# keyber/Single-Image-Super-Resolution

Measured on AMD Instinct MI355X. Metric: HR patches/sec (x2 generator fwd+bwd, LR 96x96 -> SR 192x192), higher is better.
Workload: dtype f32; 1 GPU; SRGAN x2 generator (16 blocks, 64 features, spectral norm) fwd+bwd+Adam with bicubic LR degradation and pixel-MSE x10, per-GPU batch 16 HR 192x192 patches (LR 96x96 -> SR 192x192): the north star's headline. BASELINE.json's metric string "96^2 crops, x4" is configs.cfg3 of this line. Single build: fp32.; per_gpu_batch=16, hr=192, lr=96, parallelism=dp1, hip_graph=True

## Files before the change

### single-image-super-resolution_amd/csrc/conv_trunk_f32.hip

```cpp
#include "sisr_dev.h"
#include "sisr_bf16_stage.h"
#include "sisr_instr.h"

typedef unsigned cf_u32x4 __attribute__((ext_vector_type(4)));

#include <type_traits>

#define CF_TH 8
#define CF_TW 16
#define CF_IH (CF_TH + 2)
#define CF_IW (CF_TW + 2)
#define CF_NPIX (CF_IH * CF_IW)
#define CF_PSF 36
#define CF_HALO_BYTES (CF_NPIX * CF_PSF * 4)
#define CF_WROW 36
#define CF_WCHUNK_BYTES (9 * 32 * CF_WROW * 4)
#define CF_ITEMS ((CF_NPIX * 8 + 255) / 256)
#define CF_THREADS 512
#define CF_KROWP 100
#define CF_PS 33

SISR_TRACE_BUFFER(sisr_cftrace, 512, 128)
#define CFT(k) SISR_TRACE_STAMP(sisr_cftrace, threadIdx.x == 0, blockIdx.x, k, 64, wall_clock64())
#define CFTP(k) SISR_TRACE_STAMP(sisr_cftrace, threadIdx.x == 256, blockIdx.x, 64 + (k), 128, wall_clock64())
SISR_TRACE_BUFFER(sisr_cfclk, 512, 2)
#define CFTC(k) SISR_TRACE_STAMP(sisr_cfclk, threadIdx.x == 0, blockIdx.x, (k) - 60, 2, clock64())

struct CTrunkF32Args {
    const float *x1, *x2;
    float* x_out;
    BnFinArgs fin;
    const float *pa, *pb, *pd, *ps, *pt;
    const float* slope_p; float slope;
    const float* wpk;
    const void* wimg;
    const float* bias;
    const float* res;
    float* y;
    float *stat_part, *cnt_part;
    const float *bnb_x, *bnb_scale, *bnb_shift, *bnb_mean, *bnb_invstd, *bnb_slope_p;
    float bnb_slope; int bnb_act;
    float* bnb_part;
    int N, H, W;
    int tiles_x, per_img, total, streams;
    uint32_t m_tiles_x, m_per_img;
    int glog, cout_pad, shuffle;
    int xsc, xph;
};

__device__ __forceinline__ __amdgpu_buffer_rsrc_t cf_rsrc(const void* p, unsigned bytes) {
    return __builtin_amdgcn_make_buffer_rsrc(const_cast<void*>(p), 0, (int)bytes, 0x00020000);
}

__device__ __forceinline__ void cf_split2(float v0, float v1, unsigned& hw, unsigned& lw) {
    const f32x2 v = {v0, v1};
    hw = __builtin_bit_cast(unsigned, __builtin_convertvector(v, bf16x2));
    const f32x2 r = {v0 - __uint_as_float(hw << 16), v1 - __uint_as_float(hw & 0xFFFF0000u)};
    lw = __builtin_bit_cast(unsigned, __builtin_convertvector(r, bf16x2));
}

template <int PRO, bool SPLIT>
__global__ void __launch_bounds__(CF_THREADS, 2) conv_trunk_f32_kernel(const CTrunkF32Args a) {
    extern __shared__ __attribute__((aligned(16))) unsigned char lds[];
    unsigned char* halo0 = lds + 2 * CF_WCHUNK_BYTES;
    float* red = reinterpret_cast<float*>(halo0 + 2 * CF_HALO_BYTES);

    const int tid = threadIdx.x, lane = tid & 63;
    const int wave = __builtin_amdgcn_readfirstlane(tid >> 6);
    const bool consumer = wave < 4;
    const int l31 = lane & 31, kk = lane >> 5;
    const bool xcd = (a.streams & 7) == 0;
    const int hc = xcd ? (blockIdx.x >> 3) & ((1 << a.glog) - 1) : blockIdx.x & ((1 << a.glog) - 1);
    const int stream = xcd ? (blockIdx.x & 7) | ((blockIdx.x >> (3 + a.glog)) << 3) : blockIdx.x >> a.glog;
    const unsigned tbytes = (unsigned)a.N * (unsigned)a.H * (unsigned)a.W * 256u;
    constexpr bool TWO = PRO == SISR_PRO_BNBWD || PRO == SISR_PRO_BNACT_BWD || PRO == SISR_PRO_RES_AFFINE || PRO == SISR_PRO_ACT_BWD;
    constexpr bool SUM = PRO == SISR_PRO_RES_AFFINE;
    auto tile_coords = [&](int T, int& n, int& ty, int& tx) {
        n = fdiv(T, a.m_per_img);
        const int rem = T - n * a.per_img;
        ty = fdiv(rem, a.m_tiles_x);
        tx = rem - ty * a.tiles_x;
    };

    CFT(0);
    CFTC(60);
    float* kfin = red + 4 * 32 * 3;
    const bool fin = (PRO == SISR_PRO_AFFINE_ACT || PRO == SISR_PRO_RES_AFFINE) && a.fin.stat != nullptr;
    if (fin) bn_finalize_in_kernel(a.fin, reinterpret_cast<double*>(lds), kfin, blockIdx.x == 0);
    auto fill_weights = [&]() {
        float* wl = reinterpret_cast<float*>(lds);
        if (a.wimg != nullptr) {
            constexpr int UNITS = 2 * 9 * 32 * CF_WROW / 4;
            constexpr int W_IT16 = (UNITS + CF_THREADS - 1) / CF_THREADS;
            const cf_u32x4* src = reinterpret_cast<const cf_u32x4*>(a.wimg) + hc * UNITS;
            cf_u32x4 wv16[W_IT16];
#pragma unroll
            for (int it = 0; it < W_IT16; ++it) {
                const int u = tid + it * CF_THREADS;
                wv16[it] = u < UNITS ? src[u] : cf_u32x4{0u, 0u, 0u, 0u};
            }
#pragma unroll
            for (int it = 0; it < W_IT16; ++it) {
                const int u = tid + it * CF_THREADS;
                if (u < UNITS) reinterpret_cast<cf_u32x4*>(wl)[u] = wv16[it];
            }
            return;
        }
        constexpr int W_IT = 2 * 9 * 32 * 32 / CF_THREADS;
        float wv[W_IT];
#pragma unroll
        for (int it = 0; it < W_IT; ++it) {
            const int e = tid + it * CF_THREADS;
            const int ci = e & 31, s = (e >> 5) % 3, t2 = (e >> 5) / 3;
            const int co = t2 & 31, qr = t2 >> 5;
            wv[it] = a.wpk[((int64_t)qr * a.cout_pad + 32 * hc + co) * CF_KROWP + s * CF_PS + ci];
        }
#pragma unroll
        for (int it = 0; it < W_IT; ++it) {
            const int e = tid + it * CF_THREADS;
            const int ci = e & 31, s = (e >> 5) % 3, t2 = (e >> 5) / 3;
            const int co = t2 & 31, qr = t2 >> 5;
            const int q = qr / 3, r = qr - 3 * q;
            if constexpr (SPLIT) {
                const float vo = __shfl_xor(wv[it], 1);
                const bool odd = ci & 1;
                unsigned hw, lw;
                cf_split2(odd ? vo : wv[it], odd ? wv[it] : vo, hw, lw);
                reinterpret_cast<unsigned*>(wl)[((q * 9 + r * 3 + s) * 32 + co) * CF_WROW + (odd ? 16 : 0) + (ci >> 1)] = odd ? lw : hw;
            } else {
                wl[((q * 9 + r * 3 + s) * 32 + co) * CF_WROW + ci] = wv[it];
            }
        }
    };

    const int n_mine = stream < a.total ? (a.total - stream + a.streams - 1) / a.streams : 0;
    const int n_stages = 2 * n_mine;

    if (!consumer) {
        const int pt = tid & 255, quad = tid & 7, m0 = pt >> 3;
        const int tiles_y = a.per_img / a.tiles_x;
        const float slope = PRO != SISR_PRO_NONE ? (a.slope_p ? a.slope_p[0] : a.slope) : 1.f;
        f32x4 ka[2], kb[2], kd[2], ks[2], kt[2];
        int rel[CF_ITEMS];
        unsigned flags = 0;
#pragma unroll
        for (int k = 0; k < CF_ITEMS; ++k) {
            const int px = m0 + 32 * k;
            const int py = px / CF_IW, pxx = px - py * CF_IW;
            rel[k] = ((py - 1) * a.xsc * a.xsc * a.W + (pxx - 1) * a.xsc) * 256 + quad * 16;
            const unsigned f = (py == 0 ? 1u : 0u) | (py == CF_IH - 1 ? 2u : 0u) | (pxx == 0 ? 4u : 0u) | (pxx == CF_IW - 1 ? 8u : 0u) |
                               (px >= CF_NPIX ? 16u : 0u);
            flags |= f << (5 * k);
            asm volatile("" : "+v"(rel[k]));
        }
        const bool last_beyond = m0 + 32 * (CF_ITEMS - 1) >= CF_NPIX;
        const int ldso = SPLIT ? m0 * CF_PSF * 4 + quad * 8 : (m0 * CF_PSF + quad * 4) * 4;
        const bool easy_slope = slope >= 0.f && slope <= 1.f;

        struct Stage { f32x4 s1[CF_ITEMS], s2[CF_ITEMS]; unsigned bad, origin; bool edge; };
        Stage stA, stB;
        auto issue = [&](int j, Stage& st) {
            const int T = stream + (j >> 1) * a.streams, q = j & 1;
            const unsigned xbytes = (unsigned)(a.xsc * a.xsc) * tbytes;
            const __amdgpu_buffer_rsrc_t r1 = cf_rsrc(a.x1, xbytes), r2 = cf_rsrc(TWO ? a.x2 : a.x1, xbytes);
            int n, ty, tx;
            tile_coords(T, n, ty, tx);
            const unsigned origin = (unsigned)(((n * a.xsc * a.H + a.xsc * ty * CF_TH + (a.xph >> 1)) * a.xsc * a.W + a.xsc * tx * CF_TW + (a.xph & 1)) * 256 + q * 128);
            const unsigned e = (ty == 0 ? 1u : 0u) | (ty == tiles_y - 1 ? 2u : 0u) | (tx == 0 ? 4u : 0u) | (tx == a.tiles_x - 1 ? 8u : 0u);
            st.edge = e != 0u;
            st.bad = flags & ((e | 16u) * 0x02108421u);
            st.origin = origin;
#pragma unroll
            for (int k = 0; k < CF_ITEMS; ++k) {
                const unsigned voff = origin + (unsigned)rel[k];
                st.s1[k] = __builtin_bit_cast(f32x4, __builtin_amdgcn_raw_buffer_load_b128(r1, voff, 0, 0));
                if (TWO) st.s2[k] = __builtin_bit_cast(f32x4, __builtin_amdgcn_raw_buffer_load_b128(r2, voff, 0, 0));
            }
        };
        auto commit_t = [&](auto easy_, auto edge_, int j, const Stage& st) {
            constexpr int EASY = decltype(easy_)::value;
            constexpr bool EDGE = decltype(edge_)::value;
            const int q = j & 1;
            float* img = reinterpret_cast<float*>(halo0 + (j & 1) * CF_HALO_BYTES + ldso);
            const f32x4 qa = q ? ka[1] : ka[0], qb = q ? kb[1] : kb[0], qd = q ? kd[1] : kd[0], qs = q ? ks[1] : ks[0], qt = q ? kt[1] : kt[0];
            const __amdgpu_buffer_rsrc_t ro = cf_rsrc(SUM ? a.x_out : a.x1, tbytes);
#pragma unroll
            for (int k = 0; k < CF_ITEMS; ++k) {
                if (k == CF_ITEMS - 1 && last_beyond) break;
                const bool ok = !EDGE || ((st.bad >> (5 * k)) & 31u) == 0u;
                auto value = [&](int c) {
                    const float v = st.s1[k][c];
                    if (PRO == SISR_PRO_NONE) return v;
                    if (PRO == SISR_PRO_ACT) return lrelu_t<EASY>(v, slope);
                    if (PRO == SISR_PRO_AFFINE_ACT) return lrelu_t<EASY>(qa[c] * v + qd[c], slope);
                    if (SUM) return lrelu_t<EASY>(v, slope) + (qa[c] * st.s2[k][c] + qd[c]);
                    if (PRO == SISR_PRO_ACT_BWD) return st.s2[k][c] > 0.f ? v : slope * v;
                    const float bx = st.s2[k][c];
                    float g = v;
                    if (PRO == SISR_PRO_BNACT_BWD) g = qs[c] * bx + qt[c] > 0.f ? v : slope * v;
                    return qa[c] * g + qb[c] * bx + qd[c];
                };
                const f32x4 osum = {value(0), value(1), value(2), value(3)};
                const f32x4 zero4 = {0.f, 0.f, 0.f, 0.f};
                if constexpr (SPLIT) {
                    typedef unsigned cf_u32x2 __attribute__((ext_vector_type(2)));
                    unsigned h0, l0, h1, l1;
                    cf_split2(osum[0], osum[1], h0, l0);
                    cf_split2(osum[2], osum[3], h1, l1);
                    const cf_u32x2 hw = {h0, h1}, lw = {l0, l1};
                    const cf_u32x2 z2 = {0u, 0u};
                    *reinterpret_cast<cf_u32x2*>(img + k * 32 * CF_PSF) = ok ? hw : z2;
                    *reinterpret_cast<cf_u32x2*>(img + k * 32 * CF_PSF + 16) = ok ? lw : z2;
                } else
                *reinterpret_cast<f32x4*>(img + k * 32 * CF_PSF) = ok ? osum : zero4;
                if (SUM && hc == 0 && ((flags >> (5 * k)) & 31u) == 0u)
                    __builtin_amdgcn_raw_buffer_store_b128(__builtin_bit_cast(cf_u32x4, osum), ro, st.origin + (unsigned)rel[k], 0, 0);
            }
        };
        auto commit = [&](int j, const Stage& st) {
            using T1 = std::integral_constant<int, 1>; using T0 = std::integral_constant<int, 0>;
            constexpr bool HAS_ACT = PRO == SISR_PRO_ACT || PRO == SISR_PRO_AFFINE_ACT || SUM;
            if (!HAS_ACT || easy_slope) {
                if (st.edge) commit_t(T1{}, std::true_type{}, j, st); else commit_t(T1{}, std::false_type{}, j, st);
            } else {
                if (st.edge) commit_t(T0{}, std::true_type{}, j, st); else commit_t(T0{}, std::false_type{}, j, st);
            }
        };

        issue(0, stA);
        issue(1, stB);
#pragma unroll
        for (int q = 0; q < 2; ++q)
#pragma unroll
            for (int j = 0; j < 4; ++j) {
                const int c = q * 32 + quad * 4 + j;
                constexpr bool AFF = PRO == SISR_PRO_AFFINE_ACT || (TWO && PRO != SISR_PRO_ACT_BWD);
                ka[q][j] = fin ? kfin[c] : AFF ? a.pa[c] : 1.f;
                kd[q][j] = fin ? kfin[64 + c] : AFF ? a.pd[c] : 0.f;
                kb[q][j] = (TWO && !SUM && PRO != SISR_PRO_ACT_BWD) ? a.pb[c] : 0.f;
                ks[q][j] = PRO == SISR_PRO_BNACT_BWD ? a.ps[c] : 0.f;
                kt[q][j] = PRO == SISR_PRO_BNACT_BWD ? a.pt[c] : 0.f;
            }
        fill_weights();
        __syncthreads();
        if (n_stages > 0) commit(0, stA);
        __syncthreads();
        int j = 0;
        while (j < n_stages) {
            CFTP(4 + 6 * j);
            issue(j + 2, stA);
            CFTP(5 + 6 * j);
            if (j + 1 < n_stages) commit(j + 1, stB);
            CFTP(8 + 6 * j);
            __syncthreads();
            CFTP(9 + 6 * j);
            if (++j >= n_stages) break;
            CFTP(4 + 6 * j);
            issue(j + 2, stB);
            CFTP(5 + 6 * j);
            if (j + 1 < n_stages) commit(j + 1, stA);
            CFTP(8 + 6 * j);
            __syncthreads();
            CFTP(9 + 6 * j);
            ++j;
        }
    } else {
        const int co = a.shuffle ? 32 * (hc & 1) + l31 : 32 * hc + l31;
        const int ph = hc >> 1;
        const int abase = SPLIT ? ((2 * wave + (l31 >> 4)) * CF_IW + (l31 & 15)) * CF_PSF * 4 + 16 * kk
                                : (((2 * wave + (l31 >> 4)) * CF_IW + (l31 & 15)) * CF_PSF + 16 * kk) * 4;
        const int bbase = SPLIT ? l31 * CF_WROW * 4 + 16 * kk : (l31 * CF_WROW + 16 * kk) * 4;
        const float bv = a.bias != nullptr ? a.bias[a.shuffle ? co * 4 + ph : co] : 0.f;
        float st_shift = 0.f, st_s1 = 0.f, st_s2 = 0.f;
        int st_n = 0;
        const __amdgpu_buffer_rsrc_t ry = cf_rsrc(a.y, a.shuffle ? 4u * tbytes : tbytes), rr = cf_rsrc(a.res != nullptr ? a.res : a.y, tbytes);
        f32x16 acc;
        f32x16 rv, xv;
        const bool has_x = a.bnb_part != nullptr;
        const __amdgpu_buffer_rsrc_t rxb = cf_rsrc(has_x ? a.bnb_x : a.y, tbytes);
        float b_sc = 0.f, b_sf = 0.f, b_mu = 0.f, b_is = 0.f, b_slope = 1.f;
        float rs1 = 0.f, rs2 = 0.f, rsl = 0.f;
        if (has_x) {
            b_sc = a.bnb_scale[co]; b_sf = a.bnb_shift[co]; b_mu = a.bnb_mean[co]; b_is = a.bnb_invstd[co];
            b_slope = a.bnb_slope_p ? a.bnb_slope_p[0] : a.bnb_slope;
        }
        fill_weights();
        __syncthreads();
        __syncthreads();
        for (int j = 0; j < n_stages; ++j) {
            const int q = j & 1;
            CFT(4 + 6 * j);
            int n, ty, tx;
            tile_coords(stream + (j >> 1) * a.streams, n, ty, tx);
            const unsigned obase = a.shuffle ? (unsigned)((((n * 2 * a.H + 2 * (ty * CF_TH + 2 * wave) + (ph >> 1)) * 2 * a.W + 2 * tx * CF_TW + (ph & 1)) * 64 + co) * 4)
                                             : (unsigned)((((n * a.H + ty * CF_TH + 2 * wave) * a.W + tx * CF_TW) * 64 + co) * 4);
            const int orow = a.shuffle ? 4 * a.W * 256 : a.W * 256, ocol = a.shuffle ? 512 : 256;
            if (q == 0) {
#pragma unroll
                for (int i = 0; i < 16; ++i) acc[i] = bv;
            } else {
                if (a.res != nullptr) {
#pragma unroll
                    for (int i = 0; i < 16; ++i) {
                        const int p = mfma_row(i, lane);
                        rv[i] = __builtin_bit_cast(float, __builtin_amdgcn_raw_buffer_load_b32(rr, obase + (unsigned)(((p >> 4) * a.W + (p & 15)) * 256), 0, 0));
                    }
                }
                if (has_x) {
#pragma unroll
                    for (int i = 0; i < 16; ++i) {
                        const int p = mfma_row(i, lane);
                        xv[i] = __builtin_bit_cast(float, __builtin_amdgcn_raw_buffer_load_b32(rxb, obase + (unsigned)(((p >> 4) * a.W + (p & 15)) * 256), 0, 0));
                    }
                }
            }
            const unsigned char* ab = halo0 + (j & 1) * CF_HALO_BYTES + abase;
            const unsigned char* bb = lds + q * CF_WCHUNK_BYTES + bbase;
            if constexpr (SPLIT) {
                bf16x8 ah[9][2], al[9][2], bh[9][2], bl[9][2];
                auto fetch_s = [&](int t) {
                    const unsigned char* pa = ab + ((t / 3) * CF_IW + (t % 3)) * CF_PSF * 4;
                    const unsigned char* pb = bb + t * 32 * CF_WROW * 4;
#pragma unroll
                    for (int ks = 0; ks < 2; ++ks) {
                        ah[t][ks] = *reinterpret_cast<const bf16x8*>(pa + 32 * ks);
                        bh[t][ks] = *reinterpret_cast<const bf16x8*>(pb + 32 * ks);
                        al[t][ks] = *reinterpret_cast<const bf16x8*>(pa + 64 + 32 * ks);
                        bl[t][ks] = *reinterpret_cast<const bf16x8*>(pb + 64 + 32 * ks);
                    }
                };
                fetch_s(0);
                fetch_s(1);
                __builtin_amdgcn_sched_barrier(0);
#pragma unroll
                for (int t = 0; t < 9; ++t) {
                    if (t + 2 < 9) fetch_s(t + 2);
#pragma unroll
                    for (int ks = 0; ks < 2; ++ks) {
                        acc = __builtin_amdgcn_mfma_f32_32x32x16_bf16(al[t][ks], bh[t][ks], acc, 0, 0, 0);
                        acc = __builtin_amdgcn_mfma_f32_32x32x16_bf16(ah[t][ks], bl[t][ks], acc, 0, 0, 0);
                        acc = __builtin_amdgcn_mfma_f32_32x32x16_bf16(ah[t][ks], bh[t][ks], acc, 0, 0, 0);
                    }
                    __builtin_amdgcn_sched_barrier(0);
                }
            } else {
            f32x4 af[18][2], bf[18][2];
            auto fetch = [&](int u) {
                const int t = u >> 1, s0 = 8 * (u & 1);
#pragma unroll
                for (int v = 0; v < 2; ++v) {
                    af[u][v] = *reinterpret_cast<const f32x4*>(ab + (((t / 3) * CF_IW + (t % 3)) * CF_PSF + s0 + 4 * v) * 4);
                    bf[u][v] = *reinterpret_cast<const f32x4*>(bb + ((t * 32) * CF_WROW + s0 + 4 * v) * 4);
                }
            };
            fetch(0);
            fetch(1);
            __builtin_amdgcn_sched_group_barrier(0x100, 8, 0);
#pragma unroll
            for (int u = 0; u < 18; ++u) {
                if (u + 2 < 18) fetch(u + 2);
#pragma unroll
                for (int s = 0; s < 8; ++s) acc = __builtin_amdgcn_mfma_f32_32x32x2f32(af[u][s >> 2][s & 3], bf[u][s >> 2][s & 3], acc, 0, 0, 0);
                if (u + 2 < 18) __builtin_amdgcn_sched_group_barrier(0x100, 4, 0);
                __builtin_amdgcn_sched_group_barrier(0x008, 8, 0);
            }
            }
            CFT(6 + 6 * j);
            if (q == 1) {
                if (a.res != nullptr) {
#pragma unroll
                    for (int i = 0; i < 16; ++i) acc[i] += rv[i];
                }
                if (has_x) {
                    if (a.bnb_act) {
#pragma unroll
                        for (int i = 0; i < 16; ++i) {
                            float gv = acc[i];
                            const float z = b_sc * xv[i] + b_sf;
                            const bool neg = !(z > 0.f);
                            rsl += neg ? gv * z : 0.f;
                            gv = neg ? gv * b_slope : gv;
                            rs1 += gv;
                            rs2 += gv * ((xv[i] - b_mu) * b_is);
                        }
                    } else {
#pragma unroll
                        for (int i = 0; i < 16; ++i) {
                            rs1 += acc[i];
                            rs2 += acc[i] * ((xv[i] - b_mu) * b_is);
                        }
                    }
                }
                if (a.stat_part != nullptr) {
                    if (st_n == 0) {
                        float s = 0.f;
#pragma unroll
                        for (int i = 0; i < 16; ++i) s += acc[i];
                        st_shift = s * (1.f / 16.f);
                    }
#pragma unroll
                    for (int i = 0; i < 16; ++i) {
                        const float dv = acc[i] - st_shift;
                        st_s1 += dv;
                        st_s2 += dv * dv;
                    }
                    st_n += 16;
                }
#pragma unroll
                for (int i = 0; i < 16; ++i) {
                    const int p = mfma_row(i, lane);
                    __builtin_amdgcn_raw_buffer_store_b32(__builtin_bit_cast(unsigned, (float)acc[i]), ry,
                                                          obase + (unsigned)((p >> 4) * orow + (p & 15) * ocol), 0, 0);
                }
            }
            CFT(8 + 6 * j);
            __syncthreads();
            CFT(9 + 6 * j);
        }
        CFT(3);

        if (a.stat_part != nullptr) {
            float nn = (float)st_n, mu = 0.f, m2 = 0.f;
            if (st_n > 0) {
                const float m1 = st_s1 / nn;
                mu = st_shift + m1;
                m2 = st_s2 - st_s1 * m1;
            }
            const float nb = __shfl_xor(nn, 32), mub = __shfl_xor(mu, 32), m2b = __shfl_xor(m2, 32);
            const float nt = nn + nb;
            if (nt > 0.f) { const float dl = mub - mu, f = nb / nt; mu += dl * f; m2 += m2b + dl * dl * nn * f; }
            nn = nt;
            if (kk == 0) { float* r = red + (wave * 32 + l31) * 3; r[0] = nn; r[1] = mu; r[2] = m2; }
        }
        if (has_x) {
            rs1 += __shfl_xor(rs1, 32);
            rs2 += __shfl_xor(rs2, 32);
            rsl += __shfl_xor(rsl, 32);
            if (kk == 0) { float* r = red + (wave * 32 + l31) * 3; r[0] = rs1; r[1] = rs2; r[2] = rsl; }
        }
    }
    if (a.bnb_part != nullptr) {
        __syncthreads();
        float* wk = a.bnb_part + (int64_t)blockIdx.x * 129;
        if (tid < 64) {
            const int c = tid & 31;
            const bool mine = (tid >> 5) == hc;
            float s1 = 0.f, s2 = 0.f;
            if (mine) {
                s1 = (red[c * 3] + red[(32 + c) * 3]) + (red[(64 + c) * 3] + red[(96 + c) * 3]);
                s2 = (red[c * 3 + 1] + red[(32 + c) * 3 + 1]) + (red[(64 + c) * 3 + 1] + red[(96 + c) * 3 + 1]);
            }
            wk[tid] = s1;
            wk[64 + tid] = s2;
        }
        if (tid == 64) {
            float sl = 0.f;
            for (int i = 0; i < 128; ++i) sl += red[i * 3 + 2];
            wk[128] = sl;
        }
    }
    if (a.stat_part != nullptr) {
        __syncthreads();
        if (tid < 32) {
            float nn = red[tid * 3], mm = red[tid * 3 + 1], qq = red[tid * 3 + 2];
#pragma unroll
            for (int w = 1; w < 4; ++w) {
                const float* r1 = red + (w * 32 + tid) * 3;
                const float nb = r1[0], nt = nn + nb;
                if (nt > 0.f) { const float dl = r1[1] - mm, f = nb / nt; mm += dl * f; qq += r1[2] + dl * dl * nn * f; }
                nn = nt;
            }
            float* sp = a.stat_part + (int64_t)stream * 128 + 32 * hc + tid;
            sp[0] = mm;
            sp[64] = qq;
            if (tid == 0 && hc == 0) a.cnt_part[stream] = nn;
        }
    }
    CFT(63);
    CFTC(61);
}

#include "sisr_trunk_host.h"
static const SisrTrunkKind CF_KIND = {CF_TH, CF_TW, false, 256};

int sisr_conv2d_trunk_f32_streams(const SisrConvDesc* d) {
    return sisr_equal_shares(d->N * (d->H / CF_TH) * (d->W / CF_TW), sisr_cu_slots() / (d->Cout == 256 ? 8 : 2));
}

extern "C" int sisr_conv2d_trunk_f32_eligible(const SisrConvDesc* d) {
    if (!d || sisr_switch_off("SISR_TRUNK")) return 0;
    if (sisr_switch_off("SISR_TRUNK_F32CONV")) return 0;
    if (!sisr_switch_off("SISR_TRUNK_UP") && d->Cin == 256 && d->Cout == 64 && d->KH == 3 && d->KW == 3 && d->stride == 1 && d->pad_y == 1 && d->pad_x == 1 &&
        d->x_mode == SISR_X_NHWC_UNSHUFFLE2 && d->pro_mode == SISR_PRO_ACT_BWD && d->x2 && d->y_mode == SISR_Y_NHWC && !d->x_bf16 && !d->y_bf16 &&
        !d->res_bf16 && d->Ho == d->H && d->Wo == d->W && !(d->H % CF_TH) && !(d->W % CF_TW) && d->y_sy == 1 && d->y_sx == 1 && !d->y_oy && !d->y_ox &&
        d->y_H == d->Ho && d->y_W == d->Wo && d->epi_act == SISR_EPI_NONE && d->plan.CK == 32 && d->plan.PS == CF_PS && d->plan.KROWP == CF_KROWP &&
        d->plan.CoutPad == 64 && d->plan.n_chunk == 8 && (int64_t)d->N * d->H * d->W * 1024 < (1ll << 31) &&
        d->N * (d->H / CF_TH) * (d->W / CF_TW) < 65536 && !d->stat_part && !d->bias && !d->bnb_part && !d->fin_stat)
        return 2;
    if (d->plan.CK != 32 || d->plan.PS != CF_PS || d->plan.KROWP != CF_KROWP || d->plan.n_chunk != 2 || d->plan.CoutPad != d->Cout) return 0;
    if (d->res_bf16) return 0;
    const int role = sisr_trunk_conv_role(d, CF_KIND);
    if (role == 2 && d->bnb_part && !(d->bnb_x && !d->bnbx_bf16)) return 0;
    return role;
}

template <int PRO, bool SPLIT>
static int launch_cf_t(const CTrunkF32Args& a, hipStream_t st) {
    constexpr int lds_bytes = 2 * CF_WCHUNK_BYTES + 2 * CF_HALO_BYTES + 4 * 32 * 3 * 4 + 128 * 4;
    return sisr_launch<conv_trunk_f32_kernel<PRO, SPLIT>>(dim3(a.streams << a.glog), dim3(CF_THREADS), lds_bytes, 0, st, a);
}
template <int PRO>
static int launch_cf(const CTrunkF32Args& a, bool split, hipStream_t st) {
    return split ? launch_cf_t<PRO, true>(a, st) : launch_cf_t<PRO, false>(a, st);
}

int sisr_conv2d_trunk_f32_launch(const SisrConvDesc* d, hipStream_t st) {
    CTrunkF32Args a{};
    sisr_trunk_conv_args(a, d, CF_KIND);
    const int img_mode = (d->plan.variant >> 1) & 3;
    a.wimg = (d->Cin == 64 && d->Cout == 64 && img_mode == (d->mfma_split ? 2 : 1)) ? static_cast<const void*>(d->wpk + d->plan.wpk_elems) : nullptr;
    a.streams = sisr_conv2d_trunk_f32_streams(d); a.glog = d->Cout == 256 ? 3 : 1;
    a.xsc = 1; a.xph = 0;
    if (d->Cin == 256) {
        a.xsc = 2;
        for (int ph = 0; ph < 4; ++ph) {
            a.xph = ph;
            a.wpk = d->wpk + (size_t)ph * 2 * 3 * 64 * CF_KROWP;
            a.res = ph == 0 ? d->res : d->y;
            if (int e = launch_cf<SISR_PRO_ACT_BWD>(a, d->mfma_split != 0, st)) return e;
        }
        return 0;
    }
    switch (d->pro_mode) {
        case SISR_PRO_NONE: return launch_cf<SISR_PRO_NONE>(a, d->mfma_split != 0, st);
        case SISR_PRO_ACT: return launch_cf<SISR_PRO_ACT>(a, d->mfma_split != 0, st);
        case SISR_PRO_AFFINE_ACT: return launch_cf<SISR_PRO_AFFINE_ACT>(a, d->mfma_split != 0, st);
        case SISR_PRO_BNBWD: return launch_cf<SISR_PRO_BNBWD>(a, d->mfma_split != 0, st);
        case SISR_PRO_BNACT_BWD: return launch_cf<SISR_PRO_BNACT_BWD>(a, d->mfma_split != 0, st);
        case SISR_PRO_RES_AFFINE: return launch_cf<SISR_PRO_RES_AFFINE>(a, d->mfma_split != 0, st);
    }
    return SISR_E_UNSUPPORTED;
}
```

Measured before the change: 1455 HR patches/s.

## Restructure conv trunk consumer loop with per-tile stage pairs and hoisted epilogue addressing

The consumer loop now handles one output tile per iteration, running its two weight-chunk MMA passes back to back with the chunk index as a compile-time constant. Residual and BN-input loads are issued inside the second MMA pass, after the first fragment fetches, so their latency can overlap the matrix math. Per-tile output addresses are replaced by incremental tile-coordinate stepping, a lane offset kept in a vector register, and a scalar base plus immediate offsets for the buffer loads and stores. Feature flags (residual, BN backward, stats, shuffle) are gated by template parameters so unused paths compile out. The cost is a more complex schedule that relies on `n_mine` and the stage count staying consistent with the producer side.

```diff
diff --git a/single-image-super-resolution_amd/csrc/conv_trunk_f32.hip b/single-image-super-resolution_amd/csrc/conv_trunk_f32.hip
--- a/single-image-super-resolution_amd/csrc/conv_trunk_f32.hip
+++ b/single-image-super-resolution_amd/csrc/conv_trunk_f32.hip
@@ -276,7 +276,7 @@
         const __amdgpu_buffer_rsrc_t ry = cf_rsrc(a.y, a.shuffle ? 4u * tbytes : tbytes), rr = cf_rsrc(a.res != nullptr ? a.res : a.y, tbytes);
         f32x16 acc;
         f32x16 rv, xv;
-        const bool has_x = a.bnb_part != nullptr;
+        const bool has_x = (PRO == SISR_PRO_BNBWD || PRO == SISR_PRO_BNACT_BWD) && a.bnb_part != nullptr;
         const __amdgpu_buffer_rsrc_t rxb = cf_rsrc(has_x ? a.bnb_x : a.y, tbytes);
         float b_sc = 0.f, b_sf = 0.f, b_mu = 0.f, b_is = 0.f, b_slope = 1.f;
         float rs1 = 0.f, rs2 = 0.f, rsl = 0.f;
@@ -287,35 +287,21 @@
         fill_weights();
         __syncthreads();
         __syncthreads();
-        for (int j = 0; j < n_stages; ++j) {
-            const int q = j & 1;
-            CFT(4 + 6 * j);
-            int n, ty, tx;
-            tile_coords(stream + (j >> 1) * a.streams, n, ty, tx);
-            const unsigned obase = a.shuffle ? (unsigned)((((n * 2 * a.H + 2 * (ty * CF_TH + 2 * wave) + (ph >> 1)) * 2 * a.W + 2 * tx * CF_TW + (ph & 1)) * 64 + co) * 4)
-                                             : (unsigned)((((n * a.H + ty * CF_TH + 2 * wave) * a.W + tx * CF_TW) * 64 + co) * 4);
-            const int orow = a.shuffle ? 4 * a.W * 256 : a.W * 256, ocol = a.shuffle ? 512 : 256;
-            if (q == 0) {
-#pragma unroll
-                for (int i = 0; i < 16; ++i) acc[i] = bv;
-            } else {
-                if (a.res != nullptr) {
-#pragma unroll
-                    for (int i = 0; i < 16; ++i) {
-                        const int p = mfma_row(i, lane);
-                        rv[i] = __builtin_bit_cast(float, __builtin_amdgcn_raw_buffer_load_b32(rr, obase + (unsigned)(((p >> 4) * a.W + (p & 15)) * 256), 0, 0));
-                    }
-                }
-                if (has_x) {
-#pragma unroll
-                    for (int i = 0; i < 16; ++i) {
-                        const int p = mfma_row(i, lane);
-                        xv[i] = __builtin_bit_cast(float, __builtin_amdgcn_raw_buffer_load_b32(rxb, obase + (unsigned)(((p >> 4) * a.W + (p & 15)) * 256), 0, 0));
-                    }
-                }
-            }
-            const unsigned char* ab = halo0 + (j & 1) * CF_HALO_BYTES + abase;
-            const unsigned char* bb = lds + q * CF_WCHUNK_BYTES + bbase;
+        constexpr bool BWD = TWO && !SUM;
+        const bool has_res = BWD && a.res != nullptr;
+        const bool x_act = has_x && a.bnb_act != 0;
+        const bool do_stat = !BWD && a.stat_part != nullptr;
+        const bool shuf = !TWO && a.shuffle != 0;
+        const int vl_plain = co * 4 + kk * 4 * 256, vl_shuf = co * 4 + kk * 4 * 512;
+        const int tiles_y = fdiv(a.per_img, a.m_tiles_x);
+        const int dn = fdiv(a.streams, a.m_per_img), drem = a.streams - dn * a.per_img;
+        const int dty = fdiv(drem, a.m_tiles_x), dtx = drem - dty * a.tiles_x;
+        int n, ty, tx;
+        tile_coords(stream, n, ty, tx);
+        auto mma = [&](auto q_c, auto&& mid) {
+            constexpr int Q = decltype(q_c)::value;
+            const unsigned char* ab = halo0 + Q * CF_HALO_BYTES + abase;
+            const unsigned char* bb = lds + Q * CF_WCHUNK_BYTES + bbase;
             if constexpr (SPLIT) {
                 bf16x8 ah[9][2], al[9][2], bh[9][2], bl[9][2];
                 auto fetch_s = [&](int t) {
@@ -331,6 +317,7 @@
                 };
                 fetch_s(0);
                 fetch_s(1);
+                mid();
                 __builtin_amdgcn_sched_barrier(0);
 #pragma unroll
                 for (int t = 0; t < 9; ++t) {
@@ -344,78 +331,125 @@
                     __builtin_amdgcn_sched_barrier(0);
                 }
             } else {
-            f32x4 af[18][2], bf[18][2];
-            auto fetch = [&](int u) {
-                const int t = u >> 1, s0 = 8 * (u & 1);
-#pragma unroll
-                for (int v = 0; v < 2; ++v) {
-                    af[u][v] = *reinterpret_cast<const f32x4*>(ab + (((t / 3) * CF_IW + (t % 3)) * CF_PSF + s0 + 4 * v) * 4);
-                    bf[u][v] = *reinterpret_cast<const f32x4*>(bb + ((t * 32) * CF_WROW + s0 + 4 * v) * 4);
+                f32x4 af[18][2], bf[18][2];
+                auto fetch = [&](int u) {
+                    const int t = u >> 1, s0 = 8 * (u & 1);
+#pragma unroll
+                    for (int v = 0; v < 2; ++v) {
+                        af[u][v] = *reinterpret_cast<const f32x4*>(ab + (((t / 3) * CF_IW + (t % 3)) * CF_PSF + s0 + 4 * v) * 4);
+                        bf[u][v] = *reinterpret_cast<const f32x4*>(bb + ((t * 32) * CF_WROW + s0 + 4 * v) * 4);
+                    }
+                };
+                fetch(0);
+                fetch(1);
+                __builtin_amdgcn_sched_barrier(0);
+                mid();
+                __builtin_amdgcn_sched_barrier(0);
+#pragma unroll
+                for (int u = 0; u < 18; ++u) {
+                    if (u + 2 < 18) fetch(u + 2);
+#pragma unroll
+                    for (int s = 0; s < 8; ++s) acc = __builtin_amdgcn_mfma_f32_32x32x2f32(af[u][s >> 2][s & 3], bf[u][s >> 2][s & 3], acc, 0, 0, 0);
+                    if (u + 2 < 18) __builtin_amdgcn_sched_group_barrier(0x100, 4, 0);
+                    __builtin_amdgcn_sched_group_barrier(0x008, 8, 0);
                 }
-            };
-            fetch(0);
-            fetch(1);
-            __builtin_amdgcn_sched_group_barrier(0x100, 8, 0);
-#pragma unroll
-            for (int u = 0; u < 18; ++u) {
-                if (u + 2 < 18) fetch(u + 2);
-#pragma unroll
-                for (int s = 0; s < 8; ++s) acc = __builtin_amdgcn_mfma_f32_32x32x2f32(af[u][s >> 2][s & 3], bf[u][s >> 2][s & 3], acc, 0, 0, 0);
-                if (u + 2 < 18) __builtin_amdgcn_sched_group_barrier(0x100, 4, 0);
-                __builtin_amdgcn_sched_group_barrier(0x008, 8, 0);
-            }
-            }
-            CFT(6 + 6 * j);
-            if (q == 1) {
-                if (a.res != nullptr) {
-#pragma unroll
-                    for (int i = 0; i < 16; ++i) acc[i] += rv[i];
-                }
-                if (has_x) {
-                    if (a.bnb_act) {
-#pragma unroll
-                        for (int i = 0; i < 16; ++i) {
-                            float gv = acc[i];
-                            const float z = b_sc * xv[i] + b_sf;
-                            const bool neg = !(z > 0.f);
-                            rsl += neg ? gv * z : 0.f;
-                            gv = neg ? gv * b_slope : gv;
-                            rs1 += gv;
-                            rs2 += gv * ((xv[i] - b_mu) * b_is);
-                        }
-                    } else {
-#pragma unroll
-                        for (int i = 0; i < 16; ++i) {
-                            rs1 += acc[i];
-                            rs2 += acc[i] * ((xv[i] - b_mu) * b_is);
-                        }
+            }
+        };
+        auto each_value = [&](auto ocol_c, unsigned sb, int orow, auto&& f) {
+            constexpr int OCOL = decltype(ocol_c)::value;
+            constexpr bool FAR = 11 * OCOL > 4095;
+            const unsigned s0 = sb, s1 = sb + (unsigned)orow, s0f = s0 + 8u * OCOL, s1f = s1 + 8u * OCOL;
+#pragma unroll
+            for (int i = 0; i < 16; ++i) {
+                const bool hi = (i >> 2) & 1;
+                const unsigned so = (i >> 3) ? (FAR && hi ? s1f : s1) : (FAR && hi ? s0f : s0);
+                f(i, (unsigned)(((FAR ? 0 : 8 * hi) + (i & 3)) * OCOL), so);
+            }
+        };
+        using OcolPlain = std::integral_constant<int, 256>;
+        using OcolShuf = std::integral_constant<int, 512>;
+        for (int t = 0; t < n_mine; ++t) {
+            const unsigned sb = (unsigned)(((n * a.H + ty * CF_TH + 2 * wave) * a.W + tx * CF_TW) * 256);
+            int vlp = vl_plain, vls = vl_shuf;
+            asm volatile("" : "+v"(vlp), "+v"(vls));
+            CFT(4 + 12 * t);
+            mma(std::integral_constant<int, 0>{}, [&]() {
+#pragma unroll
+                for (int i = 0; i < 16; ++i) acc[i] = bv;
+            });
+            CFT(6 + 12 * t);
+            CFT(8 + 12 * t);
+            __syncthreads();
+            CFT(9 + 12 * t);
+            CFT(10 + 12 * t);
+            mma(std::integral_constant<int, 1>{}, [&]() {
+                if (has_res)
+                    each_value(OcolPlain{}, sb, a.W * 256, [&](int i, unsigned imm, unsigned so) {
+                        rv[i] = __builtin_bit_cast(float, __builtin_amdgcn_raw_buffer_load_b32(rr, (unsigned)vlp + imm, so, 0));
+                    });
+                if (has_x)
+                    each_value(OcolPlain{}, sb, a.W * 256, [&](int i, unsigned imm, unsigned so) {
+                        xv[i] = __builtin_bit_cast(float, __builtin_amdgcn_raw_buffer_load_b32(rxb, (unsigned)vlp + imm, so, 0));
+                    });
+            });
+            CFT(12 + 12 * t);
+            if (has_res) {
+#pragma unroll
+                for (int i = 0; i < 16; ++i) acc[i] += rv[i];
+            }
+            if (has_x) {
+                if (x_act) {
+#pragma unroll
+                    for (int i = 0; i < 16; ++i) {
+                        float gv = acc[i];
+                        const float z = b_sc * xv[i] + b_sf;
+                        const bool neg = !(z > 0.f);
+                        rsl += neg ? gv * z : 0.f;
+                        gv = neg ? gv * b_slope : gv;
+                        rs1 += gv;
+                        rs2 += gv * ((xv[i] - b_mu) * b_is);
+                    }
+                } else {
+#pragma unroll
+                    for (int i = 0; i < 16; ++i) {
+                        rs1 += acc[i];
+                        rs2 += acc[i] * ((xv[i] - b_mu) * b_is);
                     }
                 }
-                if (a.stat_part != nullptr) {
-                    if (st_n == 0) {
-                        float s = 0.f;
-#pragma unroll
-                        for (int i = 0; i < 16; ++i) s += acc[i];
-                        st_shift = s * (1.f / 16.f);
-                    }
-#pragma unroll
-                    for (int i = 0; i < 16; ++i) {
-                        const float dv = acc[i] - st_shift;
-                        st_s1 += dv;
-                        st_s2 += dv * dv;
-                    }
-                    st_n += 16;
+            }
+            if (do_stat) {
+                if (st_n == 0) {
+                    float s = 0.f;
+#pragma unroll
+                    for (int i = 0; i < 16; ++i) s += acc[i];
+                    st_shift = s * (1.f / 16.f);
                 }
 #pragma unroll
                 for (int i = 0; i < 16; ++i) {
-                    const int p = mfma_row(i, lane);
-                    __builtin_amdgcn_raw_buffer_store_b32(__builtin_bit_cast(unsigned, (float)acc[i]), ry,
-                                                          obase + (unsigned)((p >> 4) * orow + (p & 15) * ocol), 0, 0);
+                    const float dv = acc[i] - st_shift;
+                    st_s1 += dv;
+                    st_s2 += dv * dv;
                 }
-            }
-            CFT(8 + 6 * j);
+                st_n += 16;
+            }
+            if (shuf) {
+                const unsigned sbs = (unsigned)(((n * 2 * a.H + 2 * (ty * CF_TH + 2 * wave) + (ph >> 1)) * 2 * a.W + 2 * tx * CF_TW + (ph & 1)) * 256);
+                each_value(OcolShuf{}, sbs, 4 * a.W * 256, [&](int i, unsigned imm, unsigned so) {
+                    __builtin_amdgcn_raw_buffer_store_b32(__builtin_bit_cast(unsigned, (float)acc[i]), ry, (unsigned)vls + imm, so, 0);
+                });
+            } else {
+                each_value(OcolPlain{}, sb, a.W * 256, [&](int i, unsigned imm, unsigned so) {
+                    __builtin_amdgcn_raw_buffer_store_b32(__builtin_bit_cast(unsigned, (float)acc[i]), ry, (unsigned)vlp + imm, so, 0);
+                });
+            }
+            CFT(14 + 12 * t);
             __syncthreads();
-            CFT(9 + 6 * j);
+            CFT(15 + 12 * t);
+            tx += dtx;
+            if (tx >= a.tiles_x) { tx -= a.tiles_x; ++ty; }
+            ty += dty;
+            if (ty >= tiles_y) { ty -= tiles_y; ++n; }
+            n += dn;
         }
         CFT(3);
 
```

New measurement: 1485 HR patches/s, median of 6. 1.02x the previous value.
